# FanmingL/Recurrent-Offpolicy-RL

Measured on NVIDIA B200. Metric: sac_update_trajectory_steps_per_s, higher is better.
Workload: dtype f32

## Files before the change

recurrent-offpolicy-rl_b200/csrc/gemm.cu:

```cuda
#include "common.cuh"
#include "tc.cuh"

namespace rorl {

constexpr int kGemmBM = 128, kGemmBN = 128, kGemmBK = 32;
constexpr int kGemmThreads = 448;
constexpr int kGemmEpiWarps = 8;
constexpr int kTileBytes = kGemmBM * kGemmBK * 4;
constexpr int kStagingBytes = kGemmEpiWarps * 32 * 128;
template <int BN, int BK = kGemmBK>
struct GemmCfg {
    static constexpr int kTileA = kGemmBM * BK * 4;
    static constexpr int kTileB = BN * BK * 4;
    static constexpr int kRaw = kTileA + kTileB;
    static constexpr int kStage = 2 * kRaw;
    static constexpr int kStages = (192 * 1024) / kStage;
    static constexpr int kSmem = kStages * kStage + kStagingBytes + 1024  + 256 ;
};

struct GemmParams {
    float* D;
    float* Dpre;
    const float* bias;
    int M, N, K, G;
// ... 245 lines not shown
                            o[j].x += bv.x; o[j].y += bv.y; o[j].z += bv.z; o[j].w += bv.w;
                        }
                    }
                    if (p.Dpre) flush(o, p.Dpre, col0);
                    if (p.act == 1) {
#pragma unroll
                        for (int j = 0; j < 8; ++j) { o[j].x = elu1(o[j].x); o[j].y = elu1(o[j].y); o[j].z = elu1(o[j].z); o[j].w = elu1(o[j].w); }
                    }
                    flush(o, p.D, col0);
                }
            }
        }
    }
    tc_fence_before();
    __syncthreads();
    if (warp == 1) {
        tc_fence_after();
        asm volatile("tcgen05.dealloc.cta_group::1.sync.aligned.b32 %0, %1;" ::"r"(tmem_base), "r"(2 * kGemmBN));
    }
}

int gemm_tn_bf16x3(const float* A, const float* B, const float* bias, float* D, float* Dpre, int64_t M, int64_t N, int64_t K, int64_t G,
                   int64_t lda, int64_t ldb, int64_t ldd, int64_t strideA, int64_t strideB, int64_t strideD,
                   int64_t strideBias, int act, int reduce_g, int transb, int single, int force_bn, void* bsplit, cudaStream_t stream);

int split_bf16_multi(const void* jobs, int njobs, cudaStream_t stream);
int gemm_nt_bf16x3(const float* A, const float* B, float* D, int64_t M, int64_t N, int64_t R, int64_t G, int64_t lda, int64_t ldb,
                   int64_t ldd, int64_t strideA, int64_t strideB, int64_t strideD, int64_t splits, int64_t strideSplit,
                   int single, cudaStream_t stream);

static int g_gemm_dbg = 0;
static int g_gemm_bn = 0;
static int g_gemm_bk = 0;
constexpr int kGemmDefaultBK = 16;
static int gemm_sms() {
    static int sms = 0;
    if (!sms) {
        int dev = 0;
        cudaGetDevice(&dev);
        cudaDeviceGetAttribute(&sms, cudaDevAttrMultiProcessorCount, dev);
        cudaFuncSetAttribute(gemm_kernel<false, 128, 32>, cudaFuncAttributeMaxDynamicSharedMemorySize, GemmCfg<128, 32>::kSmem);
        cudaFuncSetAttribute(gemm_kernel<false, 256, 32>, cudaFuncAttributeMaxDynamicSharedMemorySize, GemmCfg<256, 32>::kSmem);
        cudaFuncSetAttribute(gemm_kernel<false, 128, 16>, cudaFuncAttributeMaxDynamicSharedMemorySize, GemmCfg<128, 16>::kSmem);
        cudaFuncSetAttribute(gemm_kernel<false, 256, 16>, cudaFuncAttributeMaxDynamicSharedMemorySize, GemmCfg<256, 16>::kSmem);
        cudaFuncSetAttribute(gemm_kernel<true, 128, 32>, cudaFuncAttributeMaxDynamicSharedMemorySize, GemmCfg<128, 32>::kSmem);
    }
    return sms;
}

}

using namespace rorl;

extern "C" {

int rorl_gemm_tn(const float* A, const float* B, const float* bias, float* D, float* Dpre, int64_t M, int64_t N, int64_t K, int64_t G,
                 int64_t lda, int64_t ldb, int64_t ldd, int64_t strideA, int64_t strideB, int64_t strideD,
                 int64_t strideBias, int act, int passes, int reduce_g, int transb, void* work, cudaStream_t stream) {
    if (!A || !B || !D) return RORL_ERR_ARG;
    const bool bf = passes == 2 || passes == 4;
    if ((transb & ~3) || (transb && !bf)) return RORL_ERR_ARG;
    if ((act & ~7) || (act & 3) == 3 || ((act & 6) && !bf)) return RORL_ERR_ARG;
    if (M <= 0 || N <= 0 || K <= 0 || G <= 0) return RORL_ERR_SHAPE;
    if (K % 4 || N % 4 || lda % 4 || ldb % 4 || ldd % 4 || strideA % 4 || strideB % 4 || strideD % 4 || strideBias % 4)
        return RORL_ERR_ALIGN;
    if ((reinterpret_cast<uintptr_t>(A) | reinterpret_cast<uintptr_t>(B) | reinterpret_cast<uintptr_t>(D) |
         reinterpret_cast<uintptr_t>(bias) | reinterpret_cast<uintptr_t>(Dpre)) & 15)
        return RORL_ERR_ALIGN;
    if (passes < 1 || passes > 4) return RORL_ERR_ARG;
    if (reduce_g && (!strideA || !strideB)) return RORL_ERR_ARG;
    if (bf)
        return gemm_tn_bf16x3(A, B, bias, D, Dpre, M, N, K, G, lda, ldb, ldd, strideA, strideB, strideD, strideBias, act, reduce_g,
                              transb, passes == 4, g_gemm_bn, work, stream);
    CUtensorMap mapA, mapB;
    const bool wide = N > kGemmBN && g_gemm_bn != 128;
    const int bn = wide ? 256 : kGemmBN;
    const int bk = g_gemm_bk == 32 ? 32 : (g_gemm_bk == 16 ? 16 : kGemmDefaultBK);
    int rc = make_map(&mapA, A, M, K, lda, strideA ? G : 1, strideA, kGemmBM, bk);
    if (rc) return rc;
    rc = make_map(&mapB, B, N, K, ldb, strideB ? G : 1, strideB, bn, bk);
    if (rc) return rc;
    GemmParams p;
    p.D = D; p.Dpre = Dpre; p.bias = bias; p.M = (int)M; p.N = (int)N; p.K = (int)K; p.G = (int)G;
    p.ldd = ldd; p.strideD = strideD; p.strideBias = strideBias;
    p.a_batched = strideA != 0; p.b_batched = strideB != 0; p.act = act; p.passes = passes; p.reduce_g = reduce_g != 0;
    p.splits = 1; p.strideSplit = 0; p.dbg = g_gemm_dbg;
    const int sms = gemm_sms();
    const long long tiles = ((M + kGemmBM - 1) / kGemmBM) * ((N + bn - 1) / bn) * (reduce_g ? 1 : G);
    const int grid = (int)(tiles < sms ? tiles : sms);
    if (wide && bk == 16)
        gemm_kernel<false, 256, 16><<<grid, kGemmThreads, GemmCfg<256, 16>::kSmem, stream>>>(mapA, mapB, p);
    else if (wide)
        gemm_kernel<false, 256, 32><<<grid, kGemmThreads, GemmCfg<256, 32>::kSmem, stream>>>(mapA, mapB, p);
    else if (bk == 16)
        gemm_kernel<false, 128, 16><<<grid, kGemmThreads, GemmCfg<128, 16>::kSmem, stream>>>(mapA, mapB, p);
    else
        gemm_kernel<false, 128, 32><<<grid, kGemmThreads, GemmCfg<128, 32>::kSmem, stream>>>(mapA, mapB, p);
    RORL_RETURN_LAUNCH();
}

int rorl_split_bf16_multi(const void* jobs, int64_t njobs, cudaStream_t stream) {
    if (!jobs && njobs > 0) return RORL_ERR_ARG;
    if (njobs < 0 || njobs > 65535) return RORL_ERR_SHAPE;
    return rorl::split_bf16_multi(jobs, (int)njobs, stream);
}

int64_t rorl_gemm_tn_work_bytes(int64_t N, int64_t K, int64_t G, int64_t strideB, int passes) {
    if (passes != 2 && passes != 4) return 0;
    return 2 * (strideB ? G : 1) * N * K * 2;
}

void rorl_gemm_debug(int v) { g_gemm_dbg = v; }
void rorl_gemm_force_bn(int bn) { g_gemm_bn = bn; }
void rorl_gemm_force_bk(int bk) { g_gemm_bk = bk; }

int rorl_gemm_nt_splits(int64_t M, int64_t N, int64_t R, int64_t G) {
    if (M <= 0 || N <= 0 || R <= 0 || G <= 0) return RORL_ERR_SHAPE;
    const long long tiles = ((M + kGemmBM - 1) / kGemmBM) * ((N + kGemmBN - 1) / kGemmBN) * G;
    const long long kt = (R + kGemmBK - 1) / kGemmBK;
    long long s = (2 * 148 + tiles - 1) / tiles;
    const long long smax = kt / 4 > 0 ? kt / 4 : 1;
    if (s > smax) s = smax;
    if (s < 1) s = 1;
    return (int)s;
}

int rorl_gemm_nt(const float* A, const float* B, float* D, int64_t M, int64_t N, int64_t R, int64_t G, int64_t lda,
                 int64_t ldb, int64_t ldd, int64_t strideA, int64_t strideB, int64_t strideD, int64_t splits,
                 int64_t strideSplit, int passes, cudaStream_t stream) {
    if (!A || !B || !D) return RORL_ERR_ARG;
    if (M <= 0 || N <= 0 || R <= 0 || G <= 0 || splits <= 0) return RORL_ERR_SHAPE;
    if (M % 4 || N % 4 || lda % 4 || ldb % 4 || ldd % 4 || strideA % 4 || strideB % 4 || strideD % 4 || strideSplit % 4)
        return RORL_ERR_ALIGN;
    if ((reinterpret_cast<uintptr_t>(A) | reinterpret_cast<uintptr_t>(B) | reinterpret_cast<uintptr_t>(D)) & 15)
        return RORL_ERR_ALIGN;
    if (passes < 1 || passes > 4) return RORL_ERR_ARG;
    if (splits != rorl_gemm_nt_splits(M, N, R, G)) return RORL_ERR_ARG;
// ... 21 lines not shown
```

recurrent-offpolicy-rl_b200/csrc/gemm_bf16.cu:

```cuda
#include "common.cuh"
#include "tc.cuh"
#include <cuda_bf16.h>

namespace rorl {

constexpr int kBfBM = 128, kBfBK = 32;
#ifdef RORL_NT_MNMAJOR
constexpr bool kNtMnMajor = true;
#else
constexpr bool kNtMnMajor = false;
#endif
constexpr int kBfThreads = 448;
constexpr int kBfEpiWarps = 8;
constexpr int kBfStaging = kBfEpiWarps * 32 * 128;

template <int BN, bool MN = false>
struct BfCfg {
    static constexpr int kRawA = kBfBM * kBfBK * 4;
    static constexpr int kRaw = MN ? kRawA + BN * kBfBK * 4 : kRawA;
    static constexpr int kHalfA = kBfBM * kBfBK * 2;
    static constexpr int kHalfB = BN * kBfBK * 2;
    static constexpr int kSplit = 2 * (kHalfA + kHalfB);
    static constexpr int kRawStages = MN ? 3 : (BN == 256 ? 3 : 4);
    static constexpr int kSplitStages = MN ? 3 : (BN == 256 ? 3 : 4);
    static constexpr int kSmem = kRawStages * kRaw + kSplitStages * kSplit + kBfStaging + 1024 + 256;
};

struct BfParams {
    float* D;
    float* Dpre;
    const float* bias;
    int M, N, K, G;
    long long ldd, strideD, strideBias;
    int a_batched, b_batched, act, reduce_g;
    int accum;
    int single;
    int splits;
    long long strideSplit;
};

__device__ __forceinline__ float bf_gelu(float x) { return 0.5f * x * (1.0f + erff(x * 0.70710678118654752f)); }
__device__ __forceinline__ float bf_elu1(float x) {
    const float e = ex2f(fminf(x, 0.f) * kLog2e) - 1.0f;
    return x > 0.f ? x : e;
}

__device__ __forceinline__ void split8(const float4& a, const float4& b, uint4& hi, uint4& lo) {
    auto two = [](float x, float y, uint32_t& h, uint32_t& l) {
        const __nv_bfloat162 hh = __floats2bfloat162_rn(x, y);
        h = *reinterpret_cast<const uint32_t*>(&hh);
        const float rx = x - __uint_as_float(h << 16);
        const float ry = y - __uint_as_float(h & 0xFFFF0000u);
        const __nv_bfloat162 ll = __floats2bfloat162_rn(rx, ry);
        l = *reinterpret_cast<const uint32_t*>(&ll);
    };
    two(a.x, a.y, hi.x, lo.x);
    two(a.z, a.w, hi.y, lo.y);
    two(b.x, b.y, hi.z, lo.z);
    two(b.z, b.w, hi.w, lo.w);
}

template <int BN, bool MN, bool ACC = false>
__global__ void __launch_bounds__(kBfThreads, 1)
gemm_bf16x3_kernel(const __grid_constant__ CUtensorMap mapA, const __grid_constant__ CUtensorMap mapBhi,
                   const __grid_constant__ CUtensorMap mapBlo, const BfParams p) {
    static_assert(!MN || BN == 128, "the weight-gradient form uses 128 x 128 tiles");
    using Cfg = BfCfg<BN, MN>;
    constexpr int RS = Cfg::kRawStages, SS = Cfg::kSplitStages;
    extern __shared__ uint8_t smem_raw[];
    const uint32_t base = (smem_u32(smem_raw) + 1023u) & ~1023u;
    uint8_t* base_ptr = smem_raw + (base - smem_u32(smem_raw));
    const uint32_t split_base = base + RS * Cfg::kRaw;
    uint8_t* split_ptr = base_ptr + RS * Cfg::kRaw;
    uint8_t* staging = split_ptr + SS * Cfg::kSplit;
    const uint32_t bars = split_base + SS * Cfg::kSplit + kBfStaging;
    auto bar_raw_full = [&](int s) { return bars + 8u * s; };
    auto bar_raw_empty = [&](int s) { return bars + 8u * (RS + s); };
    auto bar_split_full = [&](int s) { return bars + 8u * (2 * RS + s); };
    auto bar_split_empty = [&](int s) { return bars + 8u * (2 * RS + SS + s); };
    auto bar_tfull = [&](int a) { return bars + 8u * (2 * RS + 2 * SS + a); };
    auto bar_tempty = [&](int a) { return bars + 8u * (2 * RS + 2 * SS + 2 + a); };
    volatile uint32_t* tmem_slot = reinterpret_cast<volatile uint32_t*>(staging + kBfStaging + 8 * (2 * RS + 2 * SS + 4));

    const int warp = threadIdx.x >> 5, lane = threadIdx.x & 31;
    const int tilesM = (p.M + kBfBM - 1) / kBfBM, tilesN = (p.N + BN - 1) / BN;
    const int KTg = (p.K + kBfBK - 1) / kBfBK;
    const int nsplit = MN ? p.splits : 1;
    const int ntiles = tilesM * tilesN * (p.reduce_g ? 1 : p.G) * nsplit;
    const int KTs = (KTg + nsplit - 1) / nsplit;
    const int KT = MN ? KTs : (p.reduce_g ? KTg * p.G : KTg);

    if (threadIdx.x == 0) {
        for (int s = 0; s < RS; ++s) {
            mbar_init(bar_raw_full(s), 1);
            mbar_init(bar_raw_empty(s), 4);
        }
        for (int s = 0; s < SS; ++s) {
            mbar_init(bar_split_full(s), MN ? 4 : 5);
            mbar_init(bar_split_empty(s), 1);
        }
        for (int a = 0; a < 2; ++a) {
            mbar_init(bar_tfull(a), 1);
            mbar_init(bar_tempty(a), kBfEpiWarps);
        }
        asm volatile("fence.mbarrier_init.release.cluster;" ::: "memory");
    }
    if (warp == 1) {
        asm volatile("tcgen05.alloc.cta_group::1.sync.aligned.shared::cta.b32 [%0], %1;" ::"r"(smem_u32((const void*)tmem_slot)), "r"(2 * BN));
        asm volatile("tcgen05.relinquish_alloc_permit.cta_group::1.sync.aligned;");
    }
    tc_fence_before();
    __syncthreads();
    tc_fence_after();
    const uint32_t tmem_base = *tmem_slot;

    if (warp == 0) {
        if (lane == 0) {
            asm volatile("prefetch.tensormap [%0];" ::"l"(&mapA) : "memory");
            asm volatile("prefetch.tensormap [%0];" ::"l"(&mapBhi) : "memory");
            asm volatile("prefetch.tensormap [%0];" ::"l"(&mapBlo) : "memory");
            uint32_t it = 0;
            for (int tile = blockIdx.x; tile < ntiles; tile += gridDim.x) {
                const int tn = tile % tilesN, tm = (tile / tilesN) % tilesM;
                const int g = (tile / (tilesN * tilesM)) % p.G;
                const int sp = tile / (tilesN * tilesM * p.G);
                for (int kt = 0; kt < KT; ++kt, ++it) {
                    const int s = it % RS, ss = it % SS;
                    const int gg = p.reduce_g ? kt / KTg : g, kk = p.reduce_g ? kt % KTg : kt;
                    mbar_wait(bar_raw_empty(s), ((it / RS) & 1) ^ 1);
                    mbar_expect_tx(bar_raw_full(s), Cfg::kRaw);
                    if (MN) {
                        const int r0 = (sp * KTs + kt) * kBfBK;
                        const uint32_t st = base + s * Cfg::kRaw;
#pragma unroll
                        for (int bI = 0; bI < 4; ++bI) {
                            tma_load_3d(st + bI * 4096, &mapA, bar_raw_full(s), tm * kBfBM + 32 * bI, r0, p.a_batched ? g : 0);
                            tma_load_3d(st + Cfg::kRawA + bI * 4096, &mapBhi, bar_raw_full(s), tn * BN + 32 * bI, r0, p.b_batched ? g : 0);
                        }
                    } else {
                        tma_load_3d(base + s * Cfg::kRaw, &mapA, bar_raw_full(s), kk * kBfBK, tm * kBfBM, p.a_batched ? gg : 0);
                        mbar_wait(bar_split_empty(ss), ((it / SS) & 1) ^ 1);
                        mbar_expect_tx(bar_split_full(ss), 2 * Cfg::kHalfB);
                        const uint32_t sb = split_base + ss * Cfg::kSplit + 2 * Cfg::kHalfA;
                        tma_load_3d(sb, &mapBhi, bar_split_full(ss), kk * kBfBK, tn * BN, p.b_batched ? gg : 0);
                        tma_load_3d(sb + Cfg::kHalfB, &mapBlo, bar_split_full(ss), kk * kBfBK, tn * BN, p.b_batched ? gg : 0);
                    }
                }
            }
        }
    } else if (warp == 1) {
        if (lane == 0) {
            const uint32_t idesc = (MN && kNtMnMajor) ? idesc_bf16_mn(kBfBM, BN) : idesc_bf16(kBfBM, BN);
            uint32_t it = 0, tcount = 0;
            for (int tile = blockIdx.x; tile < ntiles; tile += gridDim.x, ++tcount) {
                const int acc = tcount & 1;
                mbar_wait(bar_tempty(acc), ((tcount >> 1) & 1) ^ 1);
                tc_fence_after();
                const uint32_t tmem_d = tmem_base + acc * BN;
                for (int kt = 0; kt < KT; ++kt, ++it) {
                    const int s = it % SS;
                    mbar_wait(bar_split_full(s), (it / SS) & 1);
                    tc_fence_after();
                    const uint32_t st = split_base + s * Cfg::kSplit;
                    uint64_t a_hi, a_lo, b_hi, b_lo;
                    if (MN && kNtMnMajor) {
                        a_hi = make_mnmajor_desc(st, 4096, 1024); a_lo = make_mnmajor_desc(st + Cfg::kHalfA, 4096, 1024);
                        b_hi = make_mnmajor_desc(st + 2 * Cfg::kHalfA, 4096, 1024);
                        b_lo = make_mnmajor_desc(st + 2 * Cfg::kHalfA + Cfg::kHalfB, 4096, 1024);
                    } else {
                        a_hi = make_kmajor_desc_sw64(st); a_lo = make_kmajor_desc_sw64(st + Cfg::kHalfA);
                        b_hi = make_kmajor_desc_sw64(st + 2 * Cfg::kHalfA);
                        b_lo = make_kmajor_desc_sw64(st + 2 * Cfg::kHalfA + Cfg::kHalfB);
                    }
#pragma unroll
                    for (int k = 0; k < kBfBK / 16; ++k) {
                        const uint64_t adv = (MN && kNtMnMajor) ? (uint64_t)(k * 2048 >> 4) : (uint64_t)(k * 16 * 2 >> 4);
                        const uint32_t first = (kt | k) == 0 ? 0u : 1u;
                        if (!p.single) {
                            umma_bf16(tmem_d, a_lo + adv, b_hi + adv, idesc, first);
                            umma_bf16(tmem_d, a_hi + adv, b_lo + adv, idesc, 1u);
                        }
                        umma_bf16(tmem_d, a_hi + adv, b_hi + adv, idesc, p.single ? first : 1u);
                    }
                    umma_commit(bar_split_empty(s));
                }
                umma_commit(bar_tfull(acc));
            }
        }
    } else if (warp < 6) {
        const int t = threadIdx.x - 64;
        uint32_t it = 0;
        for (int tile = blockIdx.x; tile < ntiles; tile += gridDim.x) {
            for (int kt = 0; kt < KT; ++kt, ++it) {
                const int rs = it % RS, ss = it % SS;
                mbar_wait(bar_raw_full(rs), (it / RS) & 1);
                mbar_wait(bar_split_empty(ss), ((it / SS) & 1) ^ 1);
                const uint8_t* raw = base_ptr + rs * Cfg::kRaw;
                uint8_t* sp = split_ptr + ss * Cfg::kSplit;
                if (MN && kNtMnMajor) {
#pragma unroll
                    for (int op = 0; op < 2; ++op) {
                        const uint8_t* src = raw + op * Cfg::kRawA;
                        uint8_t* dhi = sp + (op ? 2 * Cfg::kHalfA : 0);
                        const int half = op ? Cfg::kHalfB : Cfg::kHalfA;
#pragma unroll
                        for (int pass = 0; pass < 4; ++pass) {
                            const int pr = pass * 16 + (t >> 3), oc = t & 7;
                            const int g = pr & 1, r = pr >> 1;
                            const int c = 2 * (oc & 3), sw = oc >> 2;
                            const uint8_t* row = src + (2 * g + sw) * 4096 + r * 128;
                            const float4 f0 = *reinterpret_cast<const float4*>(row + (((c + sw) ^ (r & 7)) << 4));
                            const float4 f1 = *reinterpret_cast<const float4*>(row + (((c + 1 - sw) ^ (r & 7)) << 4));
                            uint4 hi, lo;
                            split8(sw ? f1 : f0, sw ? f0 : f1, hi, lo);
                            uint8_t* dst = dhi + g * 4096 + r * 128 + ((oc ^ (r & 7)) << 4);
// ... 20 lines not shown
                            split8(make_float4(v[0], v[1], v[2], v[3]), make_float4(v[4], v[5], v[6], v[7]), hi, lo);
                            uint8_t* dst = drow + ((j ^ ((mn >> 1) & 3)) << 4);
                            *reinterpret_cast<uint4*>(dst) = hi;
                            *reinterpret_cast<uint4*>(dst + (op ? Cfg::kHalfB : Cfg::kHalfA)) = lo;
                        }
                    }
                } else
#pragma unroll
                for (int i = 0; i < kBfBM * 4 / 128; ++i) {
                    const int idx = t + 128 * i;
                    const int r = idx >> 2, j = idx & 3;
                    const uint8_t* src = raw + r * 128;
                    const float4 v0 = *reinterpret_cast<const float4*>(src + (((2 * j) ^ (r & 7)) << 4));
                    const float4 v1 = *reinterpret_cast<const float4*>(src + (((2 * j + 1) ^ (r & 7)) << 4));
                    uint4 hi, lo;
                    split8(v0, v1, hi, lo);
                    uint8_t* dst = sp + r * 64 + ((j ^ ((r >> 1) & 3)) << 4);
                    *reinterpret_cast<uint4*>(dst) = hi;
                    *reinterpret_cast<uint4*>(dst + Cfg::kHalfA) = lo;
                }
                asm volatile("fence.proxy.async.shared::cta;" ::: "memory");
                __syncwarp();
                if (lane == 0) {
                    mbar_arrive(bar_split_full(ss));
                    mbar_arrive(bar_raw_empty(rs));
                }
            }
        }
    } else {
        const int q = warp & 3;
        const int hf = (warp - 6) >> 2;
        uint8_t* stg = staging + (warp - 6) * 4096;
        uint32_t tcount = 0;
        for (int tile = blockIdx.x; tile < ntiles; tile += gridDim.x, ++tcount) {
            const int tn = tile % tilesN, tm = (tile / tilesN) % tilesM;
            const int g = (tile / (tilesN * tilesM)) % p.G;
            const int acc = tcount & 1;
            mbar_wait(bar_tfull(acc), (tcount >> 1) & 1);
            tc_fence_after();
            const int sp = tile / (tilesN * tilesM * p.G);
            const long long obase = (long long)g * p.strideD + (long long)sp * p.strideSplit;
            const int row0 = tm * kBfBM + q * 32;
            const float* bias = p.bias ? p.bias + (long long)g * p.strideBias : nullptr;
            auto flush = [&](const float4 (&o)[8], float* out, int col0, bool add) {
#pragma unroll
                for (int j = 0; j < 8; ++j)
                    *reinterpret_cast<float4*>(stg + lane * 128 + ((j ^ (lane & 7)) << 4)) = o[j];
                __syncwarp();
                float4 cin[ACC ? 8 : 1];
                if (ACC && add) {
#pragma unroll
                    for (int rr = 0; rr < 8; ++rr) {
                        const int grow = row0 + rr * 4 + (lane >> 3), col = col0 + (lane & 7) * 4;
                        cin[rr] = (grow < p.M && col < p.N)
                                      ? __ldcs(reinterpret_cast<const float4*>(out + obase + (long long)grow * p.ldd + col))
                                      : make_float4(0.f, 0.f, 0.f, 0.f);
                    }
                }
#pragma unroll
                for (int rr = 0; rr < 8; ++rr) {
                    const int rloc = rr * 4 + (lane >> 3), ch = lane & 7;
                    float4 v = *reinterpret_cast<const float4*>(stg + rloc * 128 + ((ch ^ (rloc & 7)) << 4));
                    const int grow = row0 + rloc, col = col0 + ch * 4;
                    if (ACC && add) { v.x += cin[ACC ? rr : 0].x; v.y += cin[ACC ? rr : 0].y; v.z += cin[ACC ? rr : 0].z; v.w += cin[ACC ? rr : 0].w; }
                    if (grow < p.M && col < p.N)
                        *reinterpret_cast<float4*>(out + obase + (long long)grow * p.ldd + col) = v;
                }
                __syncwarp();
            };
            constexpr int kHalves = BN / 128;
#pragma unroll 1
            for (int half = 0; half < kHalves; ++half) {
                const int chunk0 = (BN / 64) * hf + 2 * half;
                uint32_t r[2][32];
#pragma unroll
                for (int cc = 0; cc < 2; ++cc)
                    tmem_ld32(tmem_base + acc * BN + (chunk0 + cc) * 32 + ((uint32_t)(q * 32) << 16), r[cc]);
                tmem_ld_wait();
                if (half == kHalves - 1) {
                    tc_fence_before();
                    __syncwarp();
                    if (lane == 0) mbar_arrive(bar_tempty(acc));
                }
#pragma unroll
                for (int cc = 0; cc < 2; ++cc) {
                    const int col0 = tn * BN + (chunk0 + cc) * 32;
                    if (col0 >= p.N) break;
                    float4 o[8];
#pragma unroll
                    for (int j = 0; j < 8; ++j) {
                        o[j] = make_float4(__uint_as_float(r[cc][4 * j]), __uint_as_float(r[cc][4 * j + 1]), __uint_as_float(r[cc][4 * j + 2]),
                                           __uint_as_float(r[cc][4 * j + 3]));
                        if (bias && col0 + 4 * j < p.N) {
                            const float4 bv = __ldg(reinterpret_cast<const float4*>(bias + col0 + 4 * j));
                            o[j].x += bv.x; o[j].y += bv.y; o[j].z += bv.z; o[j].w += bv.w;
                        }
                    }
                    if (p.Dpre) flush(o, p.Dpre, col0, false);
                    if (p.act == 1) {
#pragma unroll
                        for (int j = 0; j < 8; ++j) { o[j].x = bf_elu1(o[j].x); o[j].y = bf_elu1(o[j].y); o[j].z = bf_elu1(o[j].z); o[j].w = bf_elu1(o[j].w); }
                    } else if (p.act == 2) {
#pragma unroll
                        for (int j = 0; j < 8; ++j) { o[j].x = bf_gelu(o[j].x); o[j].y = bf_gelu(o[j].y); o[j].z = bf_gelu(o[j].z); o[j].w = bf_gelu(o[j].w); }
                    }
                    flush(o, p.D, col0, p.accum != 0);
                }
            }
        }
    }
    tc_fence_before();
    __syncthreads();
    if (warp == 1) {
        tc_fence_after();
        asm volatile("tcgen05.dealloc.cta_group::1.sync.aligned.b32 %0, %1;" ::"r"(tmem_base), "r"(2 * BN));
    }
}

static int bf_sms() {
    static int sms = 0;
    if (!sms) {
        int dev = 0;
        cudaGetDevice(&dev);
        cudaDeviceGetAttribute(&sms, cudaDevAttrMultiProcessorCount, dev);
        cudaFuncSetAttribute(gemm_bf16x3_kernel<128, false>, cudaFuncAttributeMaxDynamicSharedMemorySize, BfCfg<128>::kSmem);
        cudaFuncSetAttribute(gemm_bf16x3_kernel<256, false>, cudaFuncAttributeMaxDynamicSharedMemorySize, BfCfg<256>::kSmem);
        cudaFuncSetAttribute(gemm_bf16x3_kernel<128, true>, cudaFuncAttributeMaxDynamicSharedMemorySize, BfCfg<128, true>::kSmem);
        cudaFuncSetAttribute(gemm_bf16x3_kernel<128, false, true>, cudaFuncAttributeMaxDynamicSharedMemorySize, BfCfg<128>::kSmem);
        cudaFuncSetAttribute(gemm_bf16x3_kernel<256, false, true>, cudaFuncAttributeMaxDynamicSharedMemorySize, BfCfg<256>::kSmem);
    }
    return sms;
}

__global__ void __launch_bounds__(256) split_bf16_kernel(const float* __restrict__ w, __nv_bfloat16* __restrict__ hi,
                                                         __nv_bfloat16* __restrict__ lo, int rows, int cols, long long ld, long long gs,
                                                         long long total4) {
    for (long long i = (long long)blockIdx.x * 256 + threadIdx.x; i < total4; i += (long long)gridDim.x * 256) {
        const long long e = i * 4;
        const int c = (int)(e % cols);
        const long long rg = e / cols;
        const int r = (int)(rg % rows);
        const long long g = rg / rows;
        const float4 v = *reinterpret_cast<const float4*>(w + g * gs + (long long)r * ld + c);
        const __nv_bfloat162 h0 = __floats2bfloat162_rn(v.x, v.y), h1 = __floats2bfloat162_rn(v.z, v.w);
        const uint32_t u0 = *reinterpret_cast<const uint32_t*>(&h0), u1 = *reinterpret_cast<const uint32_t*>(&h1);
        const __nv_bfloat162 l0 = __floats2bfloat162_rn(v.x - __uint_as_float(u0 << 16), v.y - __uint_as_float(u0 & 0xFFFF0000u));
        const __nv_bfloat162 l1 = __floats2bfloat162_rn(v.z - __uint_as_float(u1 << 16), v.w - __uint_as_float(u1 & 0xFFFF0000u));
        *reinterpret_cast<uint2*>(hi + e) = make_uint2(u0, u1);
        *reinterpret_cast<uint2*>(lo + e) = make_uint2(*reinterpret_cast<const uint32_t*>(&l0), *reinterpret_cast<const uint32_t*>(&l1));
    }
}

__global__ void __launch_bounds__(256) split_bf16_t_kernel(const float* __restrict__ w, __nv_bfloat16* __restrict__ hi,
                                                           __nv_bfloat16* __restrict__ lo, int N, int K, long long ld, long long gs) {
// ... 62 lines not shown

int split_bf16_multi(const void* jobs, int njobs, cudaStream_t stream) {
    if (njobs <= 0) return RORL_OK;
    dim3 grid(64u, (unsigned)njobs);
    split_bf16_multi_kernel<<<grid, 256, 0, stream>>>(reinterpret_cast<const SplitJob*>(jobs));
    RORL_RETURN_LAUNCH();
}

static int make_map_bf16(CUtensorMap* map, const void* ptr, long long rows, long long cols, long long batch, int box_rows) {
    EncodeTiledFn enc = get_encode();
    if (!enc) return RORL_ERR_ARG;
    cuuint64_t dims[3] = {(cuuint64_t)cols, (cuuint64_t)rows, (cuuint64_t)(batch > 0 ? batch : 1)};
    cuuint64_t strides[2] = {(cuuint64_t)cols * 2, (cuuint64_t)rows * cols * 2};
    cuuint32_t box[3] = {32, (cuuint32_t)box_rows, 1};
    cuuint32_t estr[3] = {1, 1, 1};
    CUresult r = enc(map, CU_TENSOR_MAP_DATA_TYPE_BFLOAT16, 3, const_cast<void*>(ptr), dims, strides, box, estr,
                     CU_TENSOR_MAP_INTERLEAVE_NONE, CU_TENSOR_MAP_SWIZZLE_64B, CU_TENSOR_MAP_L2_PROMOTION_L2_256B,
                     CU_TENSOR_MAP_FLOAT_OOB_FILL_NONE);
    return r == CUDA_SUCCESS ? RORL_OK : RORL_ERR_ARG;
}

int gemm_tn_bf16x3(const float* A, const float* B, const float* bias, float* D, float* Dpre, int64_t M, int64_t N, int64_t K, int64_t G,
                   int64_t lda, int64_t ldb, int64_t ldd, int64_t strideA, int64_t strideB, int64_t strideD,
                   int64_t strideBias, int act, int reduce_g, int transb, int single, int force_bn, void* bsplit, cudaStream_t stream) {
    if (!bsplit || (reinterpret_cast<uintptr_t>(bsplit) & 15)) return RORL_ERR_WORKSPACE;
    if (K % 8) return RORL_ERR_ALIGN;
    const int64_t GB = strideB ? G : 1;
    __nv_bfloat16* bhi = reinterpret_cast<__nv_bfloat16*>(bsplit);
    __nv_bfloat16* blo = bhi + GB * N * K;
    if (transb & 2) {
    } else if (transb & 1) {
        dim3 grid((unsigned)((N + 31) / 32), (unsigned)((K + 31) / 32), (unsigned)GB);
        split_bf16_t_kernel<<<grid, 256, 0, stream>>>(B, bhi, blo, (int)N, (int)K, ldb, strideB);
    } else {
        const long long total4 = (long long)GB * N * K / 4;
        long long nb = (total4 + 255) / 256;
        if (nb > 148 * 4) nb = 148 * 4;
        split_bf16_kernel<<<(unsigned)nb, 256, 0, stream>>>(B, bhi, blo, (int)N, (int)K, ldb, strideB, total4);
    }
    CUtensorMap mapA, mapBhi, mapBlo;
    const bool wide = N > 128 && force_bn != 128;
    const int bn = wide ? 256 : 128;
    int rc = make_map(&mapA, A, M, K, lda, strideA ? G : 1, strideA, kBfBM, kBfBK);
    if (rc) return rc;
    rc = make_map_bf16(&mapBhi, bhi, N, K, GB, bn);
    if (rc) return rc;
    rc = make_map_bf16(&mapBlo, blo, N, K, GB, bn);
    if (rc) return rc;
    BfParams p;
    p.D = D; p.Dpre = Dpre; p.bias = bias; p.M = (int)M; p.N = (int)N; p.K = (int)K; p.G = (int)G;
    p.ldd = ldd; p.strideD = strideD; p.strideBias = strideBias;
    p.a_batched = strideA != 0; p.b_batched = strideB != 0; p.act = act & 3; p.accum = (act & 4) != 0; p.reduce_g = reduce_g != 0; p.single = single != 0;
    p.splits = 1; p.strideSplit = 0;
    const int sms = bf_sms();
    const long long tiles = ((M + kBfBM - 1) / kBfBM) * ((N + bn - 1) / bn) * (reduce_g ? 1 : G);
    const int grid = (int)(tiles < sms ? tiles : sms);
    if (wide && p.accum)
        gemm_bf16x3_kernel<256, false, true><<<grid, kBfThreads, BfCfg<256>::kSmem, stream>>>(mapA, mapBhi, mapBlo, p);
    else if (p.accum)
        gemm_bf16x3_kernel<128, false, true><<<grid, kBfThreads, BfCfg<128>::kSmem, stream>>>(mapA, mapBhi, mapBlo, p);
    else if (wide)
        gemm_bf16x3_kernel<256, false><<<grid, kBfThreads, BfCfg<256>::kSmem, stream>>>(mapA, mapBhi, mapBlo, p);
    else
        gemm_bf16x3_kernel<128, false><<<grid, kBfThreads, BfCfg<128>::kSmem, stream>>>(mapA, mapBhi, mapBlo, p);
    RORL_RETURN_LAUNCH();
}

int gemm_nt_bf16x3(const float* A, const float* B, float* D, int64_t M, int64_t N, int64_t R, int64_t G, int64_t lda, int64_t ldb,
                   int64_t ldd, int64_t strideA, int64_t strideB, int64_t strideD, int64_t splits, int64_t strideSplit,
                   int single, cudaStream_t stream) {
    CUtensorMap mapA, mapB;
    int rc = make_map(&mapA, A, R, M, lda, strideA ? G : 1, strideA, kBfBK);
    if (rc) return rc;
    rc = make_map(&mapB, B, R, N, ldb, strideB ? G : 1, strideB, kBfBK);
    if (rc) return rc;
    BfParams p;
    p.D = D; p.Dpre = nullptr; p.bias = nullptr; p.M = (int)M; p.N = (int)N; p.K = (int)R; p.G = (int)G;
// ... 12 lines not shown
```

recurrent-offpolicy-rl_b200/csrc/tc.cuh:

```cuda
#pragma once
#include "common.cuh"
#include <cuda.h>

namespace rorl {

__device__ __forceinline__ void tma_load_3d(uint32_t dst, const CUtensorMap* map, uint32_t bar, int c0, int c1, int c2) {
    asm volatile(
        "cp.async.bulk.tensor.3d.shared::cluster.global.mbarrier::complete_tx::bytes [%0], [%1, {%3, %4, %5}], [%2];"
        ::"r"(dst), "l"(map), "r"(bar), "r"(c0), "r"(c1), "r"(c2) : "memory");
}
__device__ __forceinline__ void umma_tf32(uint32_t tmem_d, uint64_t adesc, uint64_t bdesc, uint32_t idesc, uint32_t accum) {
    asm volatile(
        "{\n\t.reg .pred p;\n\tsetp.ne.b32 p, %4, 0;\n\t"
        "tcgen05.mma.cta_group::1.kind::tf32 [%0], %1, %2, %3, p;\n\t}"
        ::"r"(tmem_d), "l"(adesc), "l"(bdesc), "r"(idesc), "r"(accum) : "memory");
}
__device__ __forceinline__ void umma_commit(uint32_t bar) {
    asm volatile("tcgen05.commit.cta_group::1.mbarrier::arrive::one.shared::cluster.b64 [%0];" ::"r"(bar) : "memory");
}
__device__ __forceinline__ void tc_fence_before() { asm volatile("tcgen05.fence::before_thread_sync;" ::: "memory"); }
__device__ __forceinline__ void tc_fence_after() { asm volatile("tcgen05.fence::after_thread_sync;" ::: "memory"); }

__device__ __forceinline__ uint64_t make_kmajor_desc(uint32_t saddr) {
    uint64_t d = 0;
// ... 25 lines not shown
}

__device__ __forceinline__ void umma_bf16(uint32_t tmem_d, uint64_t adesc, uint64_t bdesc, uint32_t idesc, uint32_t accum) {
    asm volatile(
        "{\n\t.reg .pred p;\n\tsetp.ne.b32 p, %4, 0;\n\t"
        "tcgen05.mma.cta_group::1.kind::f16 [%0], %1, %2, %3, p;\n\t}"
        ::"r"(tmem_d), "l"(adesc), "l"(bdesc), "r"(idesc), "r"(accum) : "memory");
}
__device__ __forceinline__ uint32_t idesc_bf16(int M, int N) {
    return (1u << 4) | (1u << 7) | (1u << 10) | ((uint32_t)(N >> 3) << 17) | ((uint32_t)(M >> 4) << 24);
}
__device__ __forceinline__ uint32_t idesc_bf16_mn(int M, int N) { return idesc_bf16(M, N) | (1u << 15) | (1u << 16); }
__device__ __forceinline__ void tmem_ld32(uint32_t taddr, uint32_t (&r)[32]) {
    asm volatile(
        "tcgen05.ld.sync.aligned.32x32b.x32.b32 "
        "{%0,%1,%2,%3,%4,%5,%6,%7,%8,%9,%10,%11,%12,%13,%14,%15,%16,%17,%18,%19,%20,%21,%22,%23,%24,%25,%26,%27,%28,%29,%30,%31}, [%32];"
        : "=r"(r[0]), "=r"(r[1]), "=r"(r[2]), "=r"(r[3]), "=r"(r[4]), "=r"(r[5]), "=r"(r[6]), "=r"(r[7]),
          "=r"(r[8]), "=r"(r[9]), "=r"(r[10]), "=r"(r[11]), "=r"(r[12]), "=r"(r[13]), "=r"(r[14]), "=r"(r[15]),
          "=r"(r[16]), "=r"(r[17]), "=r"(r[18]), "=r"(r[19]), "=r"(r[20]), "=r"(r[21]), "=r"(r[22]), "=r"(r[23]),
          "=r"(r[24]), "=r"(r[25]), "=r"(r[26]), "=r"(r[27]), "=r"(r[28]), "=r"(r[29]), "=r"(r[30]), "=r"(r[31])
        : "r"(taddr));
}
__device__ __forceinline__ void tmem_ld_wait() { asm volatile("tcgen05.wait::ld.sync.aligned;" ::: "memory"); }
__device__ __forceinline__ void fence_async_smem() { asm volatile("fence.proxy.async.shared::cta;" ::: "memory"); }

typedef CUresult (*EncodeTiledFn)(CUtensorMap*, CUtensorMapDataType, cuuint32_t, void*, const cuuint64_t*, const cuuint64_t*,
                                  const cuuint32_t*, const cuuint32_t*, CUtensorMapInterleave, CUtensorMapSwizzle,
                                  CUtensorMapL2promotion, CUtensorMapFloatOOBfill);

static inline EncodeTiledFn get_encode() {
    static EncodeTiledFn fn = nullptr;
    if (!fn) {
        void* sym = nullptr;
        cudaDriverEntryPointQueryResult qres;
        if (cudaGetDriverEntryPoint("cuTensorMapEncodeTiled", &sym, cudaEnableDefault, &qres) == cudaSuccess &&
            qres == cudaDriverEntryPointSuccess)
            fn = reinterpret_cast<EncodeTiledFn>(sym);
    }
    return fn;
}

static inline int make_map(CUtensorMap* map, const float* ptr, long long rows, long long cols, long long ld, long long batch,
                    long long batch_stride, int box_rows, int box_cols = 32) {
    EncodeTiledFn enc = get_encode();
    if (!enc) return RORL_ERR_ARG;
    cuuint64_t dims[3] = {(cuuint64_t)cols, (cuuint64_t)rows, (cuuint64_t)(batch > 0 ? batch : 1)};
// ... 26 lines not shown
```

Baseline: 2.387 million.

## Add 2-CTA cluster pair mode for the bf16x3 TN GEMM

Adds a cta_group::2 variant of the bf16x3 TN GEMM. Two CTAs in a cluster share one 256-row MMA tile, and each loads half of the B operand. Cross-CTA mbarriers, pair TMA loads and pair commits coordinate the work. The mode is on by default for N>=128 and K>=128 and can be disabled by env var or API. The aim is to halve per-CTA B traffic and shared memory and to use larger UMMA tiles, at the cost of cluster synchronization and fewer independent tiles for small M.

After: 2.403 million (median of 6 runs). About the same (+0.7%).

```diff
diff --git a/recurrent-offpolicy-rl_b200/csrc/gemm.cu b/recurrent-offpolicy-rl_b200/csrc/gemm.cu
--- a/recurrent-offpolicy-rl_b200/csrc/gemm.cu
+++ b/recurrent-offpolicy-rl_b200/csrc/gemm.cu
@@ -1,5 +1,6 @@
 #include "common.cuh"
 #include "tc.cuh"
+#include <cstdlib>
 
 namespace rorl {
 
@@ -291,7 +292,8 @@
 
 int gemm_tn_bf16x3(const float* A, const float* B, const float* bias, float* D, float* Dpre, int64_t M, int64_t N, int64_t K, int64_t G,
                    int64_t lda, int64_t ldb, int64_t ldd, int64_t strideA, int64_t strideB, int64_t strideD,
-                   int64_t strideBias, int act, int reduce_g, int transb, int single, int force_bn, void* bsplit, cudaStream_t stream);
+                   int64_t strideBias, int act, int reduce_g, int transb, int single, int force_bn, int pair_mode, void* bsplit,
+                   cudaStream_t stream);
 
 int split_bf16_multi(const void* jobs, int njobs, cudaStream_t stream);
 int gemm_nt_bf16x3(const float* A, const float* B, float* D, int64_t M, int64_t N, int64_t R, int64_t G, int64_t lda, int64_t ldb,
@@ -301,6 +303,11 @@
 static int g_gemm_dbg = 0;
 static int g_gemm_bn = 0;
 static int g_gemm_bk = 0;
+static const bool g_gemm_pair_env = [] {
+    const char* v = getenv("RORL_GEMM_PAIR");
+    return !(v && v[0] == '0');
+}();
+static int g_gemm_pair = 0;
 constexpr int kGemmDefaultBK = 16;
 static int gemm_sms() {
     static int sms = 0;
@@ -340,7 +347,8 @@
     if (reduce_g && (!strideA || !strideB)) return RORL_ERR_ARG;
     if (bf)
         return gemm_tn_bf16x3(A, B, bias, D, Dpre, M, N, K, G, lda, ldb, ldd, strideA, strideB, strideD, strideBias, act, reduce_g,
-                              transb, passes == 4, g_gemm_bn, work, stream);
+                              transb, passes == 4, g_gemm_bn, g_gemm_pair ? g_gemm_pair : (g_gemm_pair_env ? 0 : -1), work,
+                              stream);
     CUtensorMap mapA, mapB;
     const bool wide = N > kGemmBN && g_gemm_bn != 128;
     const int bn = wide ? 256 : kGemmBN;
@@ -382,6 +390,7 @@
 void rorl_gemm_debug(int v) { g_gemm_dbg = v; }
 void rorl_gemm_force_bn(int bn) { g_gemm_bn = bn; }
 void rorl_gemm_force_bk(int bk) { g_gemm_bk = bk; }
+void rorl_gemm_force_pair(int v) { g_gemm_pair = v; }
 
 int rorl_gemm_nt_splits(int64_t M, int64_t N, int64_t R, int64_t G) {
     if (M <= 0 || N <= 0 || R <= 0 || G <= 0) return RORL_ERR_SHAPE;
diff --git a/recurrent-offpolicy-rl_b200/csrc/gemm_bf16.cu b/recurrent-offpolicy-rl_b200/csrc/gemm_bf16.cu
--- a/recurrent-offpolicy-rl_b200/csrc/gemm_bf16.cu
+++ b/recurrent-offpolicy-rl_b200/csrc/gemm_bf16.cu
@@ -14,15 +14,15 @@
 constexpr int kBfEpiWarps = 8;
 constexpr int kBfStaging = kBfEpiWarps * 32 * 128;
 
-template <int BN, bool MN = false>
+template <int BN, bool MN = false, bool PAIR = false>
 struct BfCfg {
     static constexpr int kRawA = kBfBM * kBfBK * 4;
     static constexpr int kRaw = MN ? kRawA + BN * kBfBK * 4 : kRawA;
     static constexpr int kHalfA = kBfBM * kBfBK * 2;
-    static constexpr int kHalfB = BN * kBfBK * 2;
+    static constexpr int kHalfB = (PAIR ? BN / 2 : BN) * kBfBK * 2;
     static constexpr int kSplit = 2 * (kHalfA + kHalfB);
-    static constexpr int kRawStages = MN ? 3 : (BN == 256 ? 3 : 4);
-    static constexpr int kSplitStages = MN ? 3 : (BN == 256 ? 3 : 4);
+    static constexpr int kRawStages = MN ? 3 : (BN == 256 && !PAIR ? 3 : 4);
+    static constexpr int kSplitStages = MN ? 3 : (BN == 256 && !PAIR ? 3 : 4);
     static constexpr int kSmem = kRawStages * kRaw + kSplitStages * kSplit + kBfStaging + 1024 + 256;
 };
 
@@ -60,13 +60,18 @@
     two(b.z, b.w, hi.w, lo.w);
 }
 
-template <int BN, bool MN, bool ACC = false>
+template <int BN, bool MN, bool ACC = false, bool PAIR = false>
 __global__ void __launch_bounds__(kBfThreads, 1)
 gemm_bf16x3_kernel(const __grid_constant__ CUtensorMap mapA, const __grid_constant__ CUtensorMap mapBhi,
                    const __grid_constant__ CUtensorMap mapBlo, const BfParams p) {
     static_assert(!MN || BN == 128, "the weight-gradient form uses 128 x 128 tiles");
-    using Cfg = BfCfg<BN, MN>;
+    static_assert(!(MN && PAIR), "the CTA pair runs the TN form only");
+    using Cfg = BfCfg<BN, MN, PAIR>;
     constexpr int RS = Cfg::kRawStages, SS = Cfg::kSplitStages;
+    constexpr int TBM = PAIR ? 2 * kBfBM : kBfBM;
+    const uint32_t rank = PAIR ? cluster_ctarank() : 0u;
+    const int tile0 = PAIR ? (int)cluster_id_x() : (int)blockIdx.x;
+    const int tstep = PAIR ? (int)nclusters_x() : (int)gridDim.x;
     extern __shared__ uint8_t smem_raw[];
     const uint32_t base = (smem_u32(smem_raw) + 1023u) & ~1023u;
     uint8_t* base_ptr = smem_raw + (base - smem_u32(smem_raw));
@@ -83,7 +88,8 @@
     volatile uint32_t* tmem_slot = reinterpret_cast<volatile uint32_t*>(staging + kBfStaging + 8 * (2 * RS + 2 * SS + 4));
 
     const int warp = threadIdx.x >> 5, lane = threadIdx.x & 31;
-    const int tilesM = (p.M + kBfBM - 1) / kBfBM, tilesN = (p.N + BN - 1) / BN;
+    auto leader = [&](uint32_t bar) { return PAIR ? mapa_shared(bar, 0) : bar; };
+    const int tilesM = (p.M + TBM - 1) / TBM, tilesN = (p.N + BN - 1) / BN;
     const int KTg = (p.K + kBfBK - 1) / kBfBK;
     const int nsplit = MN ? p.splits : 1;
     const int ntiles = tilesM * tilesN * (p.reduce_g ? 1 : p.G) * nsplit;
@@ -96,21 +102,29 @@
             mbar_init(bar_raw_empty(s), 4);
         }
         for (int s = 0; s < SS; ++s) {
-            mbar_init(bar_split_full(s), MN ? 4 : 5);
+            mbar_init(bar_split_full(s), MN ? 4 : (PAIR ? 9 : 5));
             mbar_init(bar_split_empty(s), 1);
         }
         for (int a = 0; a < 2; ++a) {
             mbar_init(bar_tfull(a), 1);
-            mbar_init(bar_tempty(a), kBfEpiWarps);
+            mbar_init(bar_tempty(a), PAIR ? 2 * kBfEpiWarps : kBfEpiWarps);
         }
         asm volatile("fence.mbarrier_init.release.cluster;" ::: "memory");
     }
     if (warp == 1) {
-        asm volatile("tcgen05.alloc.cta_group::1.sync.aligned.shared::cta.b32 [%0], %1;" ::"r"(smem_u32((const void*)tmem_slot)), "r"(2 * BN));
-        asm volatile("tcgen05.relinquish_alloc_permit.cta_group::1.sync.aligned;");
+        if (PAIR) {
+            asm volatile("tcgen05.alloc.cta_group::2.sync.aligned.shared::cta.b32 [%0], %1;" ::"r"(smem_u32((const void*)tmem_slot)), "r"(2 * BN));
+            asm volatile("tcgen05.relinquish_alloc_permit.cta_group::2.sync.aligned;");
+        } else {
+            asm volatile("tcgen05.alloc.cta_group::1.sync.aligned.shared::cta.b32 [%0], %1;" ::"r"(smem_u32((const void*)tmem_slot)), "r"(2 * BN));
+            asm volatile("tcgen05.relinquish_alloc_permit.cta_group::1.sync.aligned;");
+        }
     }
     tc_fence_before();
-    __syncthreads();
+    if (PAIR)
+        cluster_sync();
+    else
+        __syncthreads();
     tc_fence_after();
     const uint32_t tmem_base = *tmem_slot;
 
@@ -120,7 +134,7 @@
             asm volatile("prefetch.tensormap [%0];" ::"l"(&mapBhi) : "memory");
             asm volatile("prefetch.tensormap [%0];" ::"l"(&mapBlo) : "memory");
             uint32_t it = 0;
-            for (int tile = blockIdx.x; tile < ntiles; tile += gridDim.x) {
+            for (int tile = tile0; tile < ntiles; tile += tstep) {
                 const int tn = tile % tilesN, tm = (tile / tilesN) % tilesM;
                 const int g = (tile / (tilesN * tilesM)) % p.G;
                 const int sp = tile / (tilesN * tilesM * p.G);
@@ -138,21 +152,38 @@
                             tma_load_3d(st + Cfg::kRawA + bI * 4096, &mapBhi, bar_raw_full(s), tn * BN + 32 * bI, r0, p.b_batched ? g : 0);
                         }
                     } else {
-                        tma_load_3d(base + s * Cfg::kRaw, &mapA, bar_raw_full(s), kk * kBfBK, tm * kBfBM, p.a_batched ? gg : 0);
+                        tma_load_3d(base + s * Cfg::kRaw, &mapA, bar_raw_full(s), kk * kBfBK, tm * TBM + (int)rank * kBfBM,
+                                    p.a_batched ? gg : 0);
                         mbar_wait(bar_split_empty(ss), ((it / SS) & 1) ^ 1);
-                        mbar_expect_tx(bar_split_full(ss), 2 * Cfg::kHalfB);
                         const uint32_t sb = split_base + ss * Cfg::kSplit + 2 * Cfg::kHalfA;
-                        tma_load_3d(sb, &mapBhi, bar_split_full(ss), kk * kBfBK, tn * BN, p.b_batched ? gg : 0);
-                        tma_load_3d(sb + Cfg::kHalfB, &mapBlo, bar_split_full(ss), kk * kBfBK, tn * BN, p.b_batched ? gg : 0);
+                        if (PAIR) {
+                            if (rank == 0) mbar_expect_tx(bar_split_full(ss), 4 * Cfg::kHalfB);
+                            const uint32_t fb = leader(bar_split_full(ss));
+                            const int n0 = tn * BN + (int)rank * (BN / 2);
+                            tma_load_3d_pair(sb, &mapBhi, fb, kk * kBfBK, n0, p.b_batched ? gg : 0);
+                            tma_load_3d_pair(sb + Cfg::kHalfB, &mapBlo, fb, kk * kBfBK, n0, p.b_batched ? gg : 0);
+                        } else {
+                            mbar_expect_tx(bar_split_full(ss), 2 * Cfg::kHalfB);
+                            tma_load_3d(sb, &mapBhi, bar_split_full(ss), kk * kBfBK, tn * BN, p.b_batched ? gg : 0);
+                            tma_load_3d(sb + Cfg::kHalfB, &mapBlo, bar_split_full(ss), kk * kBfBK, tn * BN, p.b_batched ? gg : 0);
+                        }
                     }
                 }
             }
         }
     } else if (warp == 1) {
-        if (lane == 0) {
-            const uint32_t idesc = (MN && kNtMnMajor) ? idesc_bf16_mn(kBfBM, BN) : idesc_bf16(kBfBM, BN);
+        if (lane == 0 && rank == 0) {
+            const uint32_t idesc = (MN && kNtMnMajor) ? idesc_bf16_mn(kBfBM, BN) : idesc_bf16(TBM, BN);
+            auto mma = [&](uint32_t d, uint64_t a, uint64_t b, uint32_t accum) {
+                if (PAIR) umma_bf16_pair(d, a, b, idesc, accum);
+                else umma_bf16(d, a, b, idesc, accum);
+            };
+            auto commit = [&](uint32_t bar) {
+                if (PAIR) umma_commit_pair(bar);
+                else umma_commit(bar);
+            };
             uint32_t it = 0, tcount = 0;
-            for (int tile = blockIdx.x; tile < ntiles; tile += gridDim.x, ++tcount) {
+            for (int tile = tile0; tile < ntiles; tile += tstep, ++tcount) {
                 const int acc = tcount & 1;
                 mbar_wait(bar_tempty(acc), ((tcount >> 1) & 1) ^ 1);
                 tc_fence_after();
@@ -177,20 +208,20 @@
                         const uint64_t adv = (MN && kNtMnMajor) ? (uint64_t)(k * 2048 >> 4) : (uint64_t)(k * 16 * 2 >> 4);
                         const uint32_t first = (kt | k) == 0 ? 0u : 1u;
                         if (!p.single) {
-                            umma_bf16(tmem_d, a_lo + adv, b_hi + adv, idesc, first);
-                            umma_bf16(tmem_d, a_hi + adv, b_lo + adv, idesc, 1u);
+                            mma(tmem_d, a_lo + adv, b_hi + adv, first);
+                            mma(tmem_d, a_hi + adv, b_lo + adv, 1u);
                         }
-                        umma_bf16(tmem_d, a_hi + adv, b_hi + adv, idesc, p.single ? first : 1u);
-                    }
-                    umma_commit(bar_split_empty(s));
-                }
-                umma_commit(bar_tfull(acc));
+                        mma(tmem_d, a_hi + adv, b_hi + adv, p.single ? first : 1u);
+                    }
+                    commit(bar_split_empty(s));
+                }
+                commit(bar_tfull(acc));
             }
         }
     } else if (warp < 6) {
         const int t = threadIdx.x - 64;
         uint32_t it = 0;
-        for (int tile = blockIdx.x; tile < ntiles; tile += gridDim.x) {
+        for (int tile = tile0; tile < ntiles; tile += tstep) {
             for (int kt = 0; kt < KT; ++kt, ++it) {
                 const int rs = it % RS, ss = it % SS;
                 mbar_wait(bar_raw_full(rs), (it / RS) & 1);
@@ -257,7 +288,8 @@
                 asm volatile("fence.proxy.async.shared::cta;" ::: "memory");
                 __syncwarp();
                 if (lane == 0) {
-                    mbar_arrive(bar_split_full(ss));
+                    if (PAIR) mbar_arrive_cluster(leader(bar_split_full(ss)));
+                    else mbar_arrive(bar_split_full(ss));
                     mbar_arrive(bar_raw_empty(rs));
                 }
             }
@@ -267,7 +299,7 @@
         const int hf = (warp - 6) >> 2;
         uint8_t* stg = staging + (warp - 6) * 4096;
         uint32_t tcount = 0;
-        for (int tile = blockIdx.x; tile < ntiles; tile += gridDim.x, ++tcount) {
+        for (int tile = tile0; tile < ntiles; tile += tstep, ++tcount) {
             const int tn = tile % tilesN, tm = (tile / tilesN) % tilesM;
             const int g = (tile / (tilesN * tilesM)) % p.G;
             const int acc = tcount & 1;
@@ -275,7 +307,7 @@
             tc_fence_after();
             const int sp = tile / (tilesN * tilesM * p.G);
             const long long obase = (long long)g * p.strideD + (long long)sp * p.strideSplit;
-            const int row0 = tm * kBfBM + q * 32;
+            const int row0 = tm * TBM + (int)rank * kBfBM + q * 32;
             const float* bias = p.bias ? p.bias + (long long)g * p.strideBias : nullptr;
             auto flush = [&](const float4 (&o)[8], float* out, int col0, bool add) {
 #pragma unroll
@@ -315,7 +347,10 @@
                 if (half == kHalves - 1) {
                     tc_fence_before();
                     __syncwarp();
-                    if (lane == 0) mbar_arrive(bar_tempty(acc));
+                    if (lane == 0) {
+                        if (PAIR) mbar_arrive_cluster(leader(bar_tempty(acc)));
+                        else mbar_arrive(bar_tempty(acc));
+                    }
                 }
 #pragma unroll
                 for (int cc = 0; cc < 2; ++cc) {
@@ -345,10 +380,16 @@
         }
     }
     tc_fence_before();
-    __syncthreads();
+    if (PAIR)
+        cluster_sync();
+    else
+        __syncthreads();
     if (warp == 1) {
         tc_fence_after();
-        asm volatile("tcgen05.dealloc.cta_group::1.sync.aligned.b32 %0, %1;" ::"r"(tmem_base), "r"(2 * BN));
+        if (PAIR)
+            asm volatile("tcgen05.dealloc.cta_group::2.sync.aligned.b32 %0, %1;" ::"r"(tmem_base), "r"(2 * BN));
+        else
+            asm volatile("tcgen05.dealloc.cta_group::1.sync.aligned.b32 %0, %1;" ::"r"(tmem_base), "r"(2 * BN));
     }
 }
 
@@ -365,6 +406,35 @@
         cudaFuncSetAttribute(gemm_bf16x3_kernel<256, false, true>, cudaFuncAttributeMaxDynamicSharedMemorySize, BfCfg<256>::kSmem);
     }
     return sms;
+}
+
+template <int BN, bool ACC>
+static int launch_pair(const CUtensorMap& mapA, const CUtensorMap& mapBhi, const CUtensorMap& mapBlo, const BfParams& p,
+                       long long tiles, cudaStream_t stream) {
+    void (*kern)(const CUtensorMap, const CUtensorMap, const CUtensorMap, const BfParams) = gemm_bf16x3_kernel<BN, false, ACC, true>;
+    constexpr int smem = BfCfg<BN, false, true>::kSmem;
+    static int clusters = 0;
+    cudaLaunchAttribute attr[1];
+    attr[0].id = cudaLaunchAttributeClusterDimension;
+    attr[0].val.clusterDim.x = 2;
+    attr[0].val.clusterDim.y = 1;
+    attr[0].val.clusterDim.z = 1;
+    cudaLaunchConfig_t cfg = {};
+    cfg.gridDim = dim3(2);
+    cfg.blockDim = dim3(kBfThreads);
+    cfg.dynamicSmemBytes = smem;
+    cfg.stream = stream;
+    cfg.attrs = attr;
+    cfg.numAttrs = 1;
+    if (!clusters) {
+        cudaError_t e = cudaFuncSetAttribute(kern, cudaFuncAttributeMaxDynamicSharedMemorySize, smem);
+        if (e == cudaSuccess) e = cudaOccupancyMaxActiveClusters(&clusters, (const void*)kern, &cfg);
+        if (e != cudaSuccess) return 1000 + (int)e;
+        if (clusters < 1) return 1000 + (int)cudaErrorInvalidConfiguration;
+    }
+    cfg.gridDim = dim3((unsigned)(2 * (tiles < clusters ? tiles : clusters)));
+    const cudaError_t e = cudaLaunchKernelEx(&cfg, kern, mapA, mapBhi, mapBlo, p);
+    return e == cudaSuccess ? RORL_OK : 1000 + (int)e;
 }
 
 __global__ void __launch_bounds__(256) split_bf16_kernel(const float* __restrict__ w, __nv_bfloat16* __restrict__ hi,
@@ -473,7 +543,8 @@
 
 int gemm_tn_bf16x3(const float* A, const float* B, const float* bias, float* D, float* Dpre, int64_t M, int64_t N, int64_t K, int64_t G,
                    int64_t lda, int64_t ldb, int64_t ldd, int64_t strideA, int64_t strideB, int64_t strideD,
-                   int64_t strideBias, int act, int reduce_g, int transb, int single, int force_bn, void* bsplit, cudaStream_t stream) {
+                   int64_t strideBias, int act, int reduce_g, int transb, int single, int force_bn, int pair_mode, void* bsplit,
+                   cudaStream_t stream) {
     if (!bsplit || (reinterpret_cast<uintptr_t>(bsplit) & 15)) return RORL_ERR_WORKSPACE;
     if (K % 8) return RORL_ERR_ALIGN;
     const int64_t GB = strideB ? G : 1;
@@ -490,13 +561,14 @@
         split_bf16_kernel<<<(unsigned)nb, 256, 0, stream>>>(B, bhi, blo, (int)N, (int)K, ldb, strideB, total4);
     }
     CUtensorMap mapA, mapBhi, mapBlo;
+    const bool pair = pair_mode > 0 || (pair_mode == 0 && N >= 128 && K >= 128);
     const bool wide = N > 128 && force_bn != 128;
     const int bn = wide ? 256 : 128;
     int rc = make_map(&mapA, A, M, K, lda, strideA ? G : 1, strideA, kBfBM, kBfBK);
     if (rc) return rc;
-    rc = make_map_bf16(&mapBhi, bhi, N, K, GB, bn);
+    rc = make_map_bf16(&mapBhi, bhi, N, K, GB, pair ? bn / 2 : bn);
     if (rc) return rc;
-    rc = make_map_bf16(&mapBlo, blo, N, K, GB, bn);
+    rc = make_map_bf16(&mapBlo, blo, N, K, GB, pair ? bn / 2 : bn);
     if (rc) return rc;
     BfParams p;
     p.D = D; p.Dpre = Dpre; p.bias = bias; p.M = (int)M; p.N = (int)N; p.K = (int)K; p.G = (int)G;
@@ -504,6 +576,13 @@
     p.a_batched = strideA != 0; p.b_batched = strideB != 0; p.act = act & 3; p.accum = (act & 4) != 0; p.reduce_g = reduce_g != 0; p.single = single != 0;
     p.splits = 1; p.strideSplit = 0;
     const int sms = bf_sms();
+    if (pair) {
+        const long long ptiles = ((M + 2 * kBfBM - 1) / (2 * kBfBM)) * ((N + bn - 1) / bn) * (reduce_g ? 1 : G);
+        if (wide && p.accum) return launch_pair<256, true>(mapA, mapBhi, mapBlo, p, ptiles, stream);
+        if (p.accum) return launch_pair<128, true>(mapA, mapBhi, mapBlo, p, ptiles, stream);
+        if (wide) return launch_pair<256, false>(mapA, mapBhi, mapBlo, p, ptiles, stream);
+        return launch_pair<128, false>(mapA, mapBhi, mapBlo, p, ptiles, stream);
+    }
     const long long tiles = ((M + kBfBM - 1) / kBfBM) * ((N + bn - 1) / bn) * (reduce_g ? 1 : G);
     const int grid = (int)(tiles < sms ? tiles : sms);
     if (wide && p.accum)
diff --git a/recurrent-offpolicy-rl_b200/csrc/tc.cuh b/recurrent-offpolicy-rl_b200/csrc/tc.cuh
--- a/recurrent-offpolicy-rl_b200/csrc/tc.cuh
+++ b/recurrent-offpolicy-rl_b200/csrc/tc.cuh
@@ -71,6 +71,48 @@
         : "r"(taddr));
 }
 __device__ __forceinline__ void tmem_ld_wait() { asm volatile("tcgen05.wait::ld.sync.aligned;" ::: "memory"); }
+
+__device__ __forceinline__ uint32_t cluster_ctarank() {
+    uint32_t r;
+    asm volatile("mov.u32 %0, %%cluster_ctarank;" : "=r"(r));
+    return r;
+}
+__device__ __forceinline__ uint32_t cluster_id_x() {
+    uint32_t r;
+    asm volatile("mov.u32 %0, %%clusterid.x;" : "=r"(r));
+    return r;
+}
+__device__ __forceinline__ uint32_t nclusters_x() {
+    uint32_t r;
+    asm volatile("mov.u32 %0, %%nclusterid.x;" : "=r"(r));
+    return r;
+}
+__device__ __forceinline__ uint32_t mapa_shared(uint32_t addr, uint32_t rank) {
+    uint32_t r;
+    asm volatile("mapa.shared::cluster.u32 %0, %1, %2;" : "=r"(r) : "r"(addr), "r"(rank));
+    return r;
+}
+__device__ __forceinline__ void mbar_arrive_cluster(uint32_t cluster_addr) {
+    asm volatile("mbarrier.arrive.shared::cluster.b64 _, [%0];" ::"r"(cluster_addr) : "memory");
+}
+__device__ __forceinline__ void cluster_sync() {
+    asm volatile("barrier.cluster.arrive.release;\n\tbarrier.cluster.wait.acquire;" ::: "memory");
+}
+__device__ __forceinline__ void tma_load_3d_pair(uint32_t dst, const CUtensorMap* map, uint32_t bar, int c0, int c1, int c2) {
+    asm volatile(
+        "cp.async.bulk.tensor.3d.cta_group::2.shared::cluster.global.mbarrier::complete_tx::bytes [%0], [%1, {%3, %4, %5}], [%2];"
+        ::"r"(dst), "l"(map), "r"(bar), "r"(c0), "r"(c1), "r"(c2) : "memory");
+}
+__device__ __forceinline__ void umma_bf16_pair(uint32_t tmem_d, uint64_t adesc, uint64_t bdesc, uint32_t idesc, uint32_t accum) {
+    asm volatile(
+        "{\n\t.reg .pred p;\n\tsetp.ne.b32 p, %4, 0;\n\t"
+        "tcgen05.mma.cta_group::2.kind::f16 [%0], %1, %2, %3, p;\n\t}"
+        ::"r"(tmem_d), "l"(adesc), "l"(bdesc), "r"(idesc), "r"(accum) : "memory");
+}
+__device__ __forceinline__ void umma_commit_pair(uint32_t bar) {
+    asm volatile("tcgen05.commit.cta_group::2.mbarrier::arrive::one.shared::cluster.multicast::cluster.b64 [%0], %1;"
+                 ::"r"(bar), "h"((uint16_t)3) : "memory");
+}
 __device__ __forceinline__ void fence_async_smem() { asm volatile("fence.proxy.async.shared::cta;" ::: "memory"); }
 
 typedef CUresult (*EncodeTiledFn)(CUtensorMap*, CUtensorMapDataType, cuuint32_t, void*, const cuuint64_t*, const cuuint64_t*,
```
